# aai-institute/USFlows

Measured on AMD Instinct MI355X. Metric: log_prob samples/sec (whole node), 32-layer 784-dim flow, batch 65536, higher is better.
Workload: dtype f32 (GEMMs as bf16x3 split on the bf16 MFMA: 24 significant bits, fp32 accumulate); 1 GPU; BASELINE cfg2: USFlow in_dims=[784], 32 additive coupling blocks, ConditionalDenseNN[256, 256]+LeakyReLU(0.01), lu_transform=1, householder=0, affine_conjugation=False, Laplace(0,1) base; log_prob of 65536 rows per GPU (65536 over 1 GPU(s)) resident in HBM; conditioned synthetic parameters (seed 100, alpha 0.1); rows_per_gpu=65536, global_rows=65536, parallelism=dp1 (single GPU: no collective), fused_coupling=True, gemm_mode=bf16x3, merge_affine=auto -> False; probe (accepted, element-wise, L1) []

## Files before the change

usflows_amd/csrc/usf_planes.hip:

```cpp
#include <stdlib.h>

#include <type_traits>

#include "usf_common.h"

namespace usf {

typedef __bf16 bf16x8 __attribute__((ext_vector_type(8)));
typedef _Float16 f16x8 __attribute__((ext_vector_type(8)));
typedef unsigned u32x4 __attribute__((ext_vector_type(4)));
#define USF_F16_GUARD 65000.0f
#define USF_PL_LOAD_A(ptr) (*(ptr))
#define USF_PL_STORE_C(v, ptr) (*(ptr) = (v))

template <int NPL> struct Planes;
template <> struct Planes<3> {
  typedef bf16x8 vec;
  static __device__ __forceinline__ f32x4 mfma(vec a, vec b, f32x4 c) { return __builtin_amdgcn_mfma_f32_16x16x32_bf16(a, b, c, 0, 0, 0); }
  static __device__ __forceinline__ void split(const float (&x)[8], vec (&o)[3]) {
#pragma unroll
    for (int j = 0; j < 8; ++j) {
      const __bf16 h = (__bf16)x[j];
      const float r = x[j] - (float)h;
      const __bf16 m = (__bf16)r;
      const float r2 = r - (float)m;
      o[0][j] = h; o[1][j] = m; o[2][j] = (__bf16)r2;
    }
  }
};
template <> struct Planes<2> {
  typedef f16x8 vec;
  static __device__ __forceinline__ f32x4 mfma(vec a, vec b, f32x4 c) { return __builtin_amdgcn_mfma_f32_16x16x32_f16(a, b, c, 0, 0, 0); }
  static __device__ __forceinline__ void split(const float (&x)[8], vec (&o)[2]) {
#pragma unroll
    for (int j = 0; j < 8; ++j) {
      const _Float16 h = (_Float16)x[j];
      const float r = x[j] - (float)h;
      o[0][j] = h; o[1][j] = (_Float16)r;
    }
  }
};

__host__ __device__ __forceinline__ int plane_feature_of_slot(int s) { return 16 * ((s & 7) >> 2) + 4 * (s >> 3) + (s & 3); }

template <int NPL>
__global__ __launch_bounds__(256) void pack_planes_kernel(const float* __restrict__ src, int64_t ld, int M, int npanels,
                                                          int nkb, const int32_t* __restrict__ idx,
                                                          const float* __restrict__ pre_div,
                                                          const float* __restrict__ pre_sub, char* __restrict__ dst,
                                                          int32_t* __restrict__ range_flag) {
  typedef Planes<NPL> PT;
  const int lane = threadIdx.x & 63;
  const int lj = lane & 15, lg = lane >> 4;
  const int64_t chunk = (int64_t)blockIdx.x * 4 + (threadIdx.x >> 6);
  if (chunk >= (int64_t)npanels * nkb) return;
  const int p = (int)(chunk / nkb), kb = (int)(chunk % nkb);
  const int row = 16 * p + lj;
  float x[8];
#pragma unroll
  for (int u = 0; u < 8; ++u) {
    const int l = 32 * kb + 16 * (u >> 2) + 4 * lg + (u & 3);
    const int c = idx[l];
    float v = 0.f;
    if (c >= 0 && row < M) {
      v = src[(int64_t)row * ld + c];
      if (pre_div) v = v / pre_div[l];
      if (pre_sub) v = v - pre_sub[l];
    }
    x[u] = v;
  }
  if (NPL == 2 && range_flag) {
    bool bad = false;
#pragma unroll
    for (int u = 0; u < 8; ++u) bad = bad || !(fabsf(x[u]) < USF_F16_GUARD);
    if (bad) atomicOr(range_flag, 1);
  }
  typename PT::vec o[NPL];
  PT::split(x, o);
  char* out = dst + (chunk * NPL) * 1024 + lane * 16;
#pragma unroll
  for (int q = 0; q < NPL; ++q) *reinterpret_cast<typename PT::vec*>(out + q * 1024) = o[q];
}

template <int NPL, bool GRAD, int NT>
__global__ __launch_bounds__(NT) void pack_planes_rows_kernel(const float* __restrict__ src, int64_t ld, int M, int nkb, int src_cols,
                                                               const int32_t* __restrict__ idx, const float* __restrict__ pre_div,
                                                               const float* __restrict__ pre_sub, char* __restrict__ dst,
                                                               int32_t* __restrict__ range_flag, const float* __restrict__ row_weight,
                                                               const float* __restrict__ loc, const float* __restrict__ scale, int grad_base,
                                                               int vec) {
  typedef Planes<NPL> PT;
  extern __shared__ float tile[];
  const int S = src_cols + 1;
  const int L = 32 * nkb;
  int* const t_idx = reinterpret_cast<int*>(tile + 16 * S);
  float* const t_div = tile + 16 * S + L;
  float* const t_sub = t_div + L;
  const int tid = threadIdx.x, lane = tid & 63, wave = tid >> 6;
  const int p = blockIdx.x;
  for (int e = tid; e < L; e += NT) {
    t_idx[e] = idx[e];
    t_div[e] = pre_div ? pre_div[e] : 1.0f;
    t_sub[e] = pre_sub ? pre_sub[e] : 0.0f;
  }
  auto xform = [&](float v, int c, float w) {
    if (!GRAD) return v;
    const float t = v - loc[c];
    const float sg = (float)((t > 0.f) - (t < 0.f));
    const float g = (grad_base == 1 + USF_BASE_LAPLACE) ? -sg / scale[c] : -t / (scale[c] * scale[c]);
    return g * w;
  };
  if (vec) {
    const int c4n = src_cols >> 2;
    for (int e = tid; e < 16 * c4n; e += NT) {
      const int r = e / c4n, c = 4 * (e - r * c4n);
      const int row = 16 * p + r;
      f32x4 v = {0.f, 0.f, 0.f, 0.f};
      float w = 0.f;
      if (row < M) {
        v = *reinterpret_cast<const f32x4*>(src + (int64_t)row * ld + c);
        if (GRAD) w = row_weight[row];
      }
#pragma unroll
      for (int q = 0; q < 4; ++q) tile[r * S + c + q] = (row < M) ? xform(v[q], c + q, w) : 0.f;
    }
    for (int e = tid; e < 16 * (src_cols & 3); e += NT) {
      const int r = e / (src_cols & 3), c = (src_cols & ~3) + e % (src_cols & 3);
      const int row = 16 * p + r;
      tile[r * S + c] = (row < M) ? xform(src[(int64_t)row * ld + c], c, GRAD ? row_weight[row] : 0.f) : 0.f;
    }
  } else {
    for (int e = tid; e < 16 * src_cols; e += NT) {
      const int r = e / src_cols, c = e - r * src_cols;
      const int row = 16 * p + r;
      tile[r * S + c] = (row < M) ? xform(src[(int64_t)row * ld + c], c, GRAD ? row_weight[row] : 0.f) : 0.f;
    }
  }
  __syncthreads();
  const int lj = lane & 15, lg = lane >> 4;
  const bool row_live = 16 * p + lj < M;
  const bool has_div = pre_div != nullptr, has_sub = pre_sub != nullptr;
  bool bad = false;
  for (int kb = wave; kb < nkb; kb += NT / 64) {
    float x[8];
#pragma unroll
    for (int u = 0; u < 8; ++u) {
      const int l = 32 * kb + 16 * (u >> 2) + 4 * lg + (u & 3);
      const int c = t_idx[l];
      float v = 0.f;
      if (c >= 0 && row_live) {
        v = tile[lj * S + c];
        if (has_div) v = v / t_div[l];
        if (has_sub) v = v - t_sub[l];
      }
      x[u] = v;
    }
    if (NPL == 2) {
#pragma unroll
      for (int u = 0; u < 8; ++u) bad = bad || !(fabsf(x[u]) < USF_F16_GUARD);
    }
    typename PT::vec o[NPL];
    PT::split(x, o);
    char* out = dst + ((int64_t)((int64_t)p * nkb + kb) * NPL) * 1024 + lane * 16;
#pragma unroll
    for (int q = 0; q < NPL; ++q) *reinterpret_cast<typename PT::vec*>(out + q * 1024) = o[q];
  }
  if (NPL == 2 && range_flag && bad) atomicOr(range_flag, 1);
}

int pack_planes(const usf_pack_planes_desc* d, hipStream_t stream) {
  if (!d) { set_error("usf_pack_planes_f32: null descriptor"); return -1; }
  if (d->M < 0 || d->nkb <= 0 || d->M > 0x7fffffff || d->nkb > 0x7fffff || d->ld < 1) { set_error("usf_pack_planes_f32: bad sizes"); return -2; }
  if (d->M == 0) return 0;
  if (!d->src || !d->idx || !d->planes) { set_error("usf_pack_planes_f32: null pointer"); return -1; }
  if (!aligned16(d->planes)) { set_error("usf_pack_planes_f32: planes must be 16-byte aligned"); return -2; }
  if (d->format != USF_PLANES_BF16X3 && d->format != USF_PLANES_F16X2) { set_error("usf_pack_planes_f32: unknown format %d", d->format); return -2; }
  const int64_t npanels = (d->M + 15) / 16;
  const int64_t chunks = npanels * d->nkb;
  const int64_t blocks = (chunks + 3) / 4;
  if (blocks > 0x7fffffffLL) { set_error("usf_pack_planes_f32: grid too large"); return -3; }
  if (d->grad_base != 0) {
    if (d->src_cols <= 0 || !d->row_weight || !d->loc || !d->scale || d->format != USF_PLANES_BF16X3 ||
        (d->grad_base != 1 + USF_BASE_LAPLACE && d->grad_base != 1 + USF_BASE_NORMAL)) {
      set_error("usf_pack_planes_f32: grad_base needs src_cols, row_weight, loc, scale, the bf16x3 format and a Laplace / Normal base");
      return -2;
    }
  }
  const int rows_env = (int)tuning("pack_rows", 1);
  const size_t lds = ((size_t)16 * (size_t)(d->src_cols + 1) + (size_t)3 * 32 * (size_t)d->nkb) * sizeof(float);
  if (d->src_cols > 0 && d->src_cols <= d->ld && lds <= 65536 && (rows_env || d->grad_base != 0)) {
    const int vec = (aligned16(d->src) && (d->ld & 3) == 0) ? 1 : 0;
    char* out = reinterpret_cast<char*>(d->planes);
    const int wide = (int)tuning("pack_wide", 1);
#define USF_PPR(NPL_, GRAD_, NT_) hipLaunchKernelGGL((pack_planes_rows_kernel<NPL_, GRAD_, NT_>), dim3((unsigned)npanels), dim3(NT_), lds, stream, \
                             d->src, d->ld, (int)d->M, (int)d->nkb, (int)d->src_cols, d->idx, d->pre_div, d->pre_sub, out, d->range_flag,  \
                             d->row_weight, d->loc, d->scale, (int)d->grad_base, vec)
#define USF_PPW(NPL_, GRAD_) do { if (wide) USF_PPR(NPL_, GRAD_, 512); else USF_PPR(NPL_, GRAD_, 256); } while (0)
    if (d->grad_base != 0) USF_PPW(3, true);
    else if (d->format == USF_PLANES_F16X2) USF_PPW(2, false);
    else USF_PPW(3, false);
#undef USF_PPW
#undef USF_PPR
    return check_launch("usf_pack_planes_f32");
  }
  if (d->grad_base != 0) { set_error("usf_pack_planes_f32: grad_base needs 16 (src_cols + 1) floats to fit 64 KB of LDS"); return -2; }
  if (d->format == USF_PLANES_F16X2)
    hipLaunchKernelGGL(pack_planes_kernel<2>, dim3((unsigned)blocks), dim3(256), 0, stream, d->src, d->ld, (int)d->M, (int)npanels,
                       (int)d->nkb, d->idx, d->pre_div, d->pre_sub, reinterpret_cast<char*>(d->planes), d->range_flag);
  else
    hipLaunchKernelGGL(pack_planes_kernel<3>, dim3((unsigned)blocks), dim3(256), 0, stream, d->src, d->ld, (int)d->M, (int)npanels,
                       (int)d->nkb, d->idx, d->pre_div, d->pre_sub, reinterpret_cast<char*>(d->planes), d->range_flag);
  return check_launch("usf_pack_planes_f32");
}

struct PlArgs {
  const char* A; const char* Wp; const float* bias; const float* post_mul;
  const char* R; char* Cp; float* Cf;
  int64_t ldc, plane_stride;
  int ldwp, wrows;
  int M, npanels;
  int a_nkb, a_kb0, nk;
  int c_nkb, c_kb0, c_kbn;
  int N, nbm, nbn, nvb;
  float res_sign, slope; int act;
  int32_t* range_flag;
  int skip_dead;
  const float* b_tab; float* b_part; int b_stride; int b_base;
  char* S; int s_kb0, s_kbn, s_both0, s_bothn;
  unsigned long long* clk;
  unsigned long long* dbg;
  unsigned long long* span;
};

template <int NPL, int TN, bool F32OUT, bool SIDE = false>
__global__ __launch_bounds__(512, 2) void gemm_planes_kernel(const PlArgs p) {
  typedef Planes<NPL> PT;
  typedef typename PT::vec vec8;
  constexpr int NT = 512;
  constexpr int BN = TN * 32;
  constexpr int FT = 2 * TN;
  constexpr unsigned CHB = NPL * 1024u;
  constexpr int CS = BN;
  constexpr int NSLOT = NPL * 4 * BN;
  constexpr int NWV = (NSLOT + NT - 1) / NT;
  constexpr int STG = NPL * 4 * CS * 4;
  constexpr int NB = 3;
  static_assert(NWV * NT - NSLOT <= NSLOT, "surplus threads wrap once");
  __shared__ __attribute__((aligned(16))) float wring[NB * STG];

  const int tid0 = threadIdx.x;
#ifdef USF_STAMP
  if (p.span && tid0 == 0) atomicMin(p.span, __builtin_amdgcn_s_memrealtime());
#endif
  unsigned long long clk_c0 = 0, clk_r0 = 0;
#ifndef USF_NO_CLOCK
  if (p.clk) { clk_c0 = __builtin_amdgcn_s_memtime(); clk_r0 = __builtin_amdgcn_s_memrealtime(); }
#endif

  for (int bid = blockIdx.x; bid < p.nvb; bid += gridDim.x) {
  int tid = tid0;
  asm volatile("" : "+v"(tid));
  const int lane = tid & 63;
  const int wave = tid >> 6;
  const int lj = lane & 15, lg = lane >> 4;
  const int xcd = bid & 7;
  const int seq = bid >> 3;
  const int pg = (seq / p.nbn) * 8 + xcd;
  const int bn = seq % p.nbn;
  if (pg >= p.nbm) continue;
  if (bid != (int)blockIdx.x) __syncthreads();
  const int n0 = bn * BN;
  int pw[2];
  pw[0] = pg * 16 + wave * 2;
  pw[1] = pw[0] + 1;

  bool dead = false;
  if (p.skip_dead && bn == p.nbn - 1 && n0 + BN <= p.wrows) {
    const int spr = 4 * p.nk;
    const int nscan = NPL * 16 * spr;
    const char* const wz = p.Wp + 2 * ((int64_t)(n0 + BN - 16) * p.ldwp);
    unsigned nz = 0;
    for (int e0 = tid; e0 < nscan; e0 += 4 * NT) {
      u32x4 v[4];
#pragma unroll
      for (int i = 0; i < 4; ++i) {
        const int e = min(e0 + i * NT, nscan - 1);
        const int pl = e / (16 * spr), rem = e - pl * (16 * spr);
        const int r = rem / spr, c = rem - r * spr;
        v[i] = *reinterpret_cast<const u32x4*>(wz + 2 * (pl * p.plane_stride + (int64_t)r * p.ldwp + 8 * c));
      }
#pragma unroll
      for (int i = 0; i < 4; ++i) nz |= v[i][0] | v[i][1] | v[i][2] | v[i][3];
    }
    dead = __builtin_amdgcn_readfirstlane(__syncthreads_or(nz != 0)) == 0;
  }
  auto tile = [&](auto dead_c) {
  unsigned aoff[2];
#pragma unroll
  for (int b = 0; b < 2; ++b)
    aoff[b] = ((unsigned)min(pw[b], p.npanels - 1) * (unsigned)p.a_nkb + (unsigned)p.a_kb0) * CHB + (unsigned)lane * 16u;
  auto issue_a = [&](int kb, vec8 (&dst)[2][NPL]) {
#pragma unroll
    for (int b = 0; b < 2; ++b)
#pragma unroll
      for (int q = 0; q < NPL; ++q)
        dst[b][q] = USF_PL_LOAD_A(reinterpret_cast<const vec8*>(p.A + (aoff[b] + (unsigned)kb * CHB + (unsigned)q * 1024u)));
  };

  unsigned wsrc[NWV];
  int wdst[NWV];
#pragma unroll
  for (int i = 0; i < NWV; ++i) {
    const int idx = tid + NT * i;
    const int idc = (idx < NSLOT) ? idx : idx - NSLOT;
    const int pl = idc / (4 * BN), rem = idc % (4 * BN);
    const int r = rem >> 2, ch = rem & 3;
    wsrc[i] = (unsigned)(2 * (pl * p.plane_stride + (int64_t)min(n0 + r, p.wrows - 1) * p.ldwp + 8 * ch));
    wdst[i] = 4 * ((pl * 4 + ch) * CS + (r ^ (2 * ch)));
  }
  auto issue_w = [&](int k0, f32x4 (&dst)[NWV]) {
#pragma unroll
    for (int i = 0; i < NWV; ++i) dst[i] = *reinterpret_cast<const f32x4*>(p.Wp + (wsrc[i] + 2u * (unsigned)k0));
  };
  auto store_w = [&](float* wb, const f32x4 (&src)[NWV]) {
#pragma unroll
    for (int i = 0; i < NWV; ++i) *reinterpret_cast<f32x4*>(wb + wdst[i]) = src[i];
  };

  f32x4 acc[FT][2];
  const f32x4 zero4 = {0.f, 0.f, 0.f, 0.f};
#pragma unroll
  for (int ft = 0; ft < FT; ++ft) {
    f32x4 bv = zero4;
    if (p.bias) bv = *reinterpret_cast<const f32x4*>(p.bias + min(n0 + ft * 16 + 4 * lg, p.wrows - 4));
    acc[ft][0] = bv;
    acc[ft][1] = bv;
  }

#ifdef USF_STAMP
#define PSTAMP(v) unsigned long long v = __builtin_amdgcn_s_memtime(); __builtin_amdgcn_sched_barrier(0)
#else
#define PSTAMP(v)
#endif
  PSTAMP(t0);
#ifdef USF_STAMP
  const unsigned long long rt0 = __builtin_amdgcn_s_memrealtime();
#endif
  vec8 pa[2][NPL], pb[2][NPL];
  vec8 fr[2][NPL], f2[2][NPL];
  f32x4 wst[NWV];
  const int nslab = p.nk;
  auto ks = [&](int s_) { return s_; };
  issue_w(ks(0) * 32, wst);
  store_w(wring, wst);
  issue_a(ks(0), pa);
  issue_w(ks(min(1, nslab - 1)) * 32, wst);
  __syncthreads();
  const float* const wl0 = wring + 4 * (lg * CS + (lj ^ (2 * lg)));
  auto read_pair = [&](const float* wl, int pr, vec8 (&f)[2][NPL]) {
#pragma unroll
    for (int q = 0; q < NPL; ++q) {
      f[0][q] = *reinterpret_cast<const vec8*>(wl + 4 * (q * 4 * CS + (2 * pr) * 16));
      f[1][q] = *reinterpret_cast<const vec8*>(wl + 4 * (q * 4 * CS + (2 * pr + 1) * 16));
    }
  };
  auto read_half = [&](const float* wl, int pr, vec8 (&f)[2][NPL]) {
#pragma unroll
    for (int q = 0; q < NPL; ++q) f[0][q] = *reinterpret_cast<const vec8*>(wl + 4 * (q * 4 * CS + (2 * pr) * 16));
  };
  read_pair(wl0, 0, fr);

  constexpr int NPR = (NPL == 3) ? 6 : 3;
  constexpr int NP = TN;
  constexpr int MID = (NP - 1) / 2;
  constexpr int NLD = 2 * NPL;
  constexpr int LPP = (NLD + MID) / (MID + 1);
#define USF_MM(FT_, W, P)                                        \
  acc[FT_][0] = PT::mfma(W, cur[0][P], acc[FT_][0]);             \
  acc[FT_][1] = PT::mfma(W, cur[1][P], acc[FT_][1])
  static_assert(NP - 1 > MID + 1, "the last pair runs behind the barrier and carries no global loads");
  auto mm_pair = [&](auto dead_c, int pr, const vec8 (&f)[2][NPL], const vec8 (&cur)[2][NPL]) {
    const int ft = 2 * pr;
    if (decltype(dead_c)::value && pr == NP - 1) {
      if constexpr (NPL == 3) {
        USF_MM(ft, f[0][2], 0); USF_MM(ft, f[0][1], 1); USF_MM(ft, f[0][0], NPL - 1); USF_MM(ft, f[0][1], 0);
        USF_MM(ft, f[0][0], 1); USF_MM(ft, f[0][0], 0);
      } else {
        USF_MM(ft, f[0][1], 0); USF_MM(ft, f[0][0], 1); USF_MM(ft, f[0][0], 0);
      }
    } else if constexpr (NPL == 3) {
      USF_MM(ft, f[0][2], 0); USF_MM(ft + 1, f[1][2], 0); USF_MM(ft, f[0][1], 1); USF_MM(ft + 1, f[1][1], 1);
      USF_MM(ft, f[0][0], NPL - 1); USF_MM(ft + 1, f[1][0], NPL - 1); USF_MM(ft, f[0][1], 0); USF_MM(ft + 1, f[1][1], 0);
      USF_MM(ft, f[0][0], 1); USF_MM(ft + 1, f[1][0], 1); USF_MM(ft, f[0][0], 0); USF_MM(ft + 1, f[1][0], 0);
    } else {
      USF_MM(ft, f[0][1], 0); USF_MM(ft + 1, f[1][1], 0); USF_MM(ft, f[0][0], 1); USF_MM(ft + 1, f[1][0], 1);
      USF_MM(ft, f[0][0], 0); USF_MM(ft + 1, f[1][0], 0);
    }
  };
#if defined(USF_STAMP) && USF_STAMP >= 2
  unsigned long long ph[4] = {0, 0, 0, 0};
#define LSTAMP(v) PSTAMP(v)
#define LACC(i, a, b) ph[i] += (b) - (a)
#else
#define LSTAMP(v)
#define LACC(i, a, b)
#endif
  auto slab = [&](auto dead_c, int s, int ring_s, const vec8 (&cur)[2][NPL], vec8 (&nxt)[2][NPL], vec8 (&fA)[2][NPL], vec8 (&fB)[2][NPL]) {
    constexpr bool DEAD = decltype(dead_c)::value;
    LSTAMP(l0);
    const int ring_n = (ring_s == 2) ? 0 : ring_s + 1;
    const float* wl = wl0 + ring_s * STG;
    const float* wln = wl0 + ring_n * STG;
    auto read_next = [&](int pr, vec8 (&f)[2][NPL]) {
      if (DEAD && pr + 1 == NP - 1) read_half(wl, pr + 1, f); else read_pair(wl, pr + 1, f);
    };
    float* wb = wring + ring_n * STG;
    issue_a(ks(min(s + 1, nslab - 1)), nxt);
#pragma unroll
    for (int pr = 0; pr <= MID; ++pr) {
      if (pr & 1) { if (pr + 1 < NP) read_next(pr, fA); mm_pair(dead_c, pr, fB, cur); }
      else        { if (pr + 1 < NP) read_next(pr, fB); mm_pair(dead_c, pr, fA, cur); }
      if (pr == MID) store_w(wb, wst);
      __builtin_amdgcn_sched_group_barrier(0x100, 2 * NPL, 0);
      if (pr < MID) {
        __builtin_amdgcn_sched_group_barrier(0x008, 2 * NPR, 0);
        if (pr * LPP < NLD) __builtin_amdgcn_sched_group_barrier(0x020, LPP, 0);
        __builtin_amdgcn_sched_group_barrier(0x008, 2 * NPR, 0);
      } else {
        constexpr int MPS = (4 * NPR) / (NWV + 1);
#pragma unroll
        for (int i = 0; i < NWV; ++i) {
          __builtin_amdgcn_sched_group_barrier(0x008, MPS, 0);
          __builtin_amdgcn_sched_group_barrier(0x200, 1, 0);
        }
        __builtin_amdgcn_sched_group_barrier(0x008, 4 * NPR - NWV * MPS, 0);
      }
    }
    __builtin_amdgcn_sched_barrier(0);
    LSTAMP(l1);
    LSTAMP(l2);
    __syncthreads();
    __builtin_amdgcn_sched_barrier(0);
    LSTAMP(l3);
    issue_w(ks(min(s + 2, nslab - 1)) * 32, wst);
#pragma unroll
    for (int pr = MID + 1; pr < NP; ++pr) {
      if (pr & 1) { if (pr + 1 < NP) read_next(pr, fA); else read_pair(wln, 0, fA); mm_pair(dead_c, pr, fB, cur); }
      else        { if (pr + 1 < NP) read_next(pr, fB); else read_pair(wln, 0, fB); mm_pair(dead_c, pr, fA, cur); }
      if (DEAD && pr + 1 == NP - 1) __builtin_amdgcn_sched_group_barrier(0x100, NPL, 0);
      else __builtin_amdgcn_sched_group_barrier(0x100, 2 * NPL, 0);
      if (pr == MID + 1) {
        __builtin_amdgcn_sched_group_barrier(0x008, 2 * NPR, 0);
        __builtin_amdgcn_sched_group_barrier(0x020, NWV, 0);
        __builtin_amdgcn_sched_group_barrier(0x008, 2 * NPR, 0);
      } else if (DEAD && pr == NP - 1) {
        __builtin_amdgcn_sched_group_barrier(0x008, 2 * NPR, 0);
      } else {
        __builtin_amdgcn_sched_group_barrier(0x008, 4 * NPR, 0);
      }
    }
    __builtin_amdgcn_sched_barrier(0);
    LSTAMP(l4);
    LACC(0, l0, l1); LACC(1, l1, l2); LACC(2, l2, l3); LACC(3, l3, l4);
  };
  PSTAMP(t1);
    int s = 0, ring = 0;
    for (; s + 2 <= nslab; s += 2) {
      slab(dead_c, s, ring, pa, pb, fr, f2);
      ring = (ring == 2) ? 0 : ring + 1;
      if (NP & 1) slab(dead_c, s + 1, ring, pb, pa, f2, fr); else slab(dead_c, s + 1, ring, pb, pa, fr, f2);
      ring = (ring == 2) ? 0 : ring + 1;
    }
    if (s < nslab) slab(dead_c, s, ring, pa, pb, fr, f2);
  PSTAMP(t2);

  bool bad = false;
  if (p.act == USF_ACT_LEAKY_RELU) {
#pragma unroll
    for (int ft = 0; ft < FT; ++ft)
#pragma unroll
      for (int b = 0; b < 2; ++b)
#pragma unroll
        for (int j = 0; j < 4; ++j) acc[ft][b][j] = act_apply(acc[ft][b][j], USF_ACT_LEAKY_RELU, p.slope);
  }
  if (F32OUT) {
    const bool vec_ok = ((p.ldc & 3) == 0) && ((reinterpret_cast<uintptr_t>(p.Cf) & 15u) == 0);
#pragma unroll
    for (int b = 0; b < 2; ++b) {
      const int row = 16 * pw[b] + lj;
      float bsum = 0.f;
#pragma unroll
      for (int ft = 0; ft < FT; ++ft) {
        const int col = n0 + 16 * ft + 4 * lg;
        f32x4 v = acc[ft][b];
        if (p.post_mul) v = v * *reinterpret_cast<const f32x4*>(p.post_mul + min(col, p.wrows - 4));
        if (p.b_part) {
          const float* t = p.b_tab + min(col, p.b_stride - 4);
          const f32x4 bl = *reinterpret_cast<const f32x4*>(t);
          const f32x4 bi = *reinterpret_cast<const f32x4*>(t + p.b_stride);
          const f32x4 bc = *reinterpret_cast<const f32x4*>(t + 2 * p.b_stride);
#pragma unroll
          for (int j = 0; j < 4; ++j) {
            const float d = (v[j] - bl[j]) * bi[j];
            const float term = (p.b_base == USF_BASE_LAPLACE) ? bc[j] - fabsf(d) : bc[j] - 0.5f * d * d;
            bsum += (col + j < p.N) ? term : 0.f;
          }
        }
        if (NPL == 2 && row < p.M && col < p.N) {
#pragma unroll
          for (int j = 0; j < 4; ++j) bad = bad || (col + j < p.N && !(fabsf(v[j]) < 3.0e38f));
        }
        if (p.Cf != nullptr && row < p.M && col < p.N) {
          float* dst = p.Cf + (int64_t)row * p.ldc + col;
          if (vec_ok && col + 3 < p.N) {
            *reinterpret_cast<f32x4*>(dst) = v;
          } else {
#pragma unroll
            for (int j = 0; j < 4; ++j)
              if (col + j < p.N) dst[j] = v[j];
          }
        }
      }
      if (p.b_part) {
        bsum += __shfl_xor(bsum, 16);
        bsum += __shfl_xor(bsum, 32);
        if (lg == 0 && row < p.M) p.b_part[(int64_t)row * 8 + bn] = bsum;
      }
    }
  } else {
#pragma unroll
    for (int t = 0; t < TN; ++t) {
      const int kbo = bn * TN + t;
      const bool to_side = SIDE && (unsigned)(kbo - p.s_kb0) < (unsigned)p.s_kbn;
      const bool to_planes = !to_side || (unsigned)(kbo - p.s_both0) < (unsigned)p.s_bothn;
#pragma unroll
      for (int b = 0; b < 2; ++b) {
        if (kbo < p.c_kbn && pw[b] < p.npanels) {
          const size_t off = (((size_t)pw[b] * p.c_nkb + (p.c_kb0 + kbo)) * NPL) * 1024 + (size_t)lane * 16;
          float x[8];
#pragma unroll
          for (int u = 0; u < 8; ++u) x[u] = acc[2 * t + (u >> 2)][b][u & 3];
          if constexpr (SIDE) {
            if (to_side) {
              const unsigned soff = ((unsigned)pw[b] * (unsigned)p.s_kbn + (unsigned)(kbo - p.s_kb0)) * 2048u + (unsigned)lane * 32u;
              f32x4 s0 = {x[0], x[1], x[2], x[3]}, s1 = {x[4], x[5], x[6], x[7]};
              if constexpr (NPL == 2) {
                bool sb = false;
#pragma unroll
                for (int u = 0; u < 8; ++u) sb = sb || (16 * pw[b] + lj < p.M && !(fabsf(x[u]) < USF_F16_GUARD));
                bad = bad || sb;
                vec8 so[NPL];
                PT::split(x, so);
#pragma unroll
                for (int u = 0; u < 4; ++u) {
                  s0[u] = (float)so[0][u] + (float)so[1][u];
                  s1[u] = (float)so[0][4 + u] + (float)so[1][4 + u];
                }
              }
              *reinterpret_cast<f32x4*>(p.S + soff) = s0;
              *reinterpret_cast<f32x4*>(p.S + (soff + 16u)) = s1;
            }
            if (!to_planes) continue;
          }
          if (p.R) {
            vec8 r[NPL];
#pragma unroll
            for (int q = 0; q < NPL; ++q) r[q] = *reinterpret_cast<const vec8*>(p.R + off + q * 1024);
#pragma unroll
            for (int u = 0; u < 8; ++u) {
              float rv = (float)r[0][u] + (float)r[1][u];
              if (NPL == 3) rv = rv + (float)r[NPL - 1][u];
              x[u] = rv + p.res_sign * x[u];
            }
          }
          if (NPL == 2) {
#pragma unroll
            for (int u = 0; u < 8; ++u) bad = bad || (16 * pw[b] + lj < p.M && !(fabsf(x[u]) < USF_F16_GUARD));
          }
          vec8 o[NPL];
          PT::split(x, o);
#ifdef USF_NOSTORE
          if (o[0][0] == (decltype(o[0][0] + o[0][0]))1234.5f && o[1][1] == (decltype(o[0][0] + o[0][0]))77.f)
#endif
          {
#pragma unroll
            for (int q = 0; q < NPL; ++q) USF_PL_STORE_C(o[q], reinterpret_cast<vec8*>(p.Cp + off + q * 1024));
          }
        }
      }
    }
  }
  if (NPL == 2 && p.range_flag && bad) atomicOr(p.range_flag, 1);
#ifdef USF_STAMP
  PSTAMP(t3);
  if (p.dbg && lane == 0) {
    unsigned long long* o = p.dbg + (size_t)((bid % 2048) * 8 + wave) * 8;
    o[0] = t1 - t0; o[1] = t2 - t1; o[2] = t3 - t2; o[3] = t3 - t0; o[4] = 1; o[5] = __builtin_amdgcn_s_memrealtime() - rt0;
    o[6] = rt0; o[7] = __builtin_amdgcn_s_memrealtime();
#if USF_STAMP >= 2
    unsigned long long* o2 = p.dbg + 16384 * 8 + (size_t)((bid % 2048) * 8 + wave) * 8;
    for (int i = 0; i < 4; ++i) o2[i] = ph[i];
#endif
  }
#endif
  };
  if (dead) tile(std::true_type()); else tile(std::false_type());
#undef USF_MM
  }
#ifdef USF_STAMP
  if (p.span && tid0 == 0) atomicMax(p.span + 1, __builtin_amdgcn_s_memrealtime());
#endif
#ifndef USF_NO_CLOCK
  if (p.clk && tid0 == 0) {
    atomicAdd(p.clk, __builtin_amdgcn_s_memtime() - clk_c0);
    atomicAdd(p.clk + 1, __builtin_amdgcn_s_memrealtime() - clk_r0);
  }
#endif
}

#ifdef USF_STAMP
unsigned long long* g_pdbg = nullptr;
unsigned long long* g_pspan = nullptr;
#endif

template <int NPL, int TN>
static int launch_planes(PlArgs a, bool f32out, hipStream_t stream) {
  const bool side = a.S != nullptr;
  constexpr int BN = TN * 32;
  a.nbm = (a.npanels + 15) / 16;
  a.nbn = f32out ? (a.N + BN - 1) / BN : (a.c_kbn + TN - 1) / TN;
  int64_t grid = (((int64_t)a.nbm + 7) / 8) * 8 * a.nbn;
  if (grid > 0x7fffffffLL) { set_error("usf_gemm_planes: grid too large"); return -3; }
  a.nvb = (int)grid;
  const int persist = (int)tuning("planes_persist", 1);
  int cus = device_cu_count();
  cus = (cus / 8) * 8 > 0 ? (cus / 8) * 8 : 8;
  if (persist && grid > cus) grid = cus;
  if (f32out) hipLaunchKernelGGL((gemm_planes_kernel<NPL, TN, true>), dim3((unsigned)grid), dim3(512), 0, stream, a);
  else if (side) hipLaunchKernelGGL((gemm_planes_kernel<NPL, TN, false, true>), dim3((unsigned)grid), dim3(512), 0, stream, a);
  else hipLaunchKernelGGL((gemm_planes_kernel<NPL, TN, false>), dim3((unsigned)grid), dim3(512), 0, stream, a);
  return check_launch("usf_gemm_planes");
}

int gemm_planes_tn(int64_t nblk) {
  const int64_t pad5 = (nblk + 4) / 5 * 5 - nblk, pad4 = (nblk + 3) / 4 * 4 - nblk;
  return pad4 < pad5 ? 4 : 5;
}

int gemm_planes_variant(const usf_gemm_planes_desc* d) {
  if (!d || d->M <= 0) return 0;
  const bool f32out = d->C_f32 != nullptr || d->base_part != nullptr;
  const int64_t nblk = f32out ? (d->N + 31) / 32 : d->c_kbn;
  if (nblk <= 0) return 0;
  return 5000 + 10 * gemm_planes_tn(nblk) + (f32out ? 1 : 0);
}

int gemm_planes_side(const usf_gemm_planes_desc* d, void* side, int64_t side_kb0, int64_t side_kbn, int64_t both_kb0,
                     int64_t both_kbn, hipStream_t stream) {
  if (!d) { set_error("usf_gemm_planes_bf16x3: null descriptor"); return -1; }
  if (d->M < 0 || d->M > 0x7fffffff || d->nk <= 0 || d->a_nkb <= 0 || d->a_kb0 < 0 || d->a_kb0 + d->nk > d->a_nkb ||
      d->w_rows < 4 || d->w_rows > 0x7fffffff) {
    set_error("usf_gemm_planes_bf16x3: bad sizes (M=%lld nk=%lld a_nkb=%lld a_kb0=%lld w_rows=%lld)", (long long)d->M,
              (long long)d->nk, (long long)d->a_nkb, (long long)d->a_kb0, (long long)d->w_rows);
    return -2;
  }
  if (d->M == 0) return 0;
  const bool f32out = d->C_f32 != nullptr || d->base_part != nullptr;
  if (!d->A || !d->W_planes || (!f32out && !d->C_planes)) { set_error("usf_gemm_planes_bf16x3: null A / W / C"); return -1; }
  if (f32out && d->C_planes) { set_error("usf_gemm_planes_bf16x3: give C_planes or C_f32, not both"); return -2; }
  if (!aligned16(d->A) || !aligned16(d->W_planes) || (d->C_planes && !aligned16(d->C_planes)) ||
      (d->residual && !aligned16(d->residual)) || (d->bias && !aligned16(d->bias)) || (d->post_mul && !aligned16(d->post_mul))) {
    set_error("usf_gemm_planes_bf16x3: pointers must be 16-byte aligned");
    return -2;
  }
  if ((d->ldw & 7) || d->ldw < 32 * d->nk || (d->w_rows & 3)) { set_error("usf_gemm_planes_bf16x3: ldw must be a multiple of 8 and >= 32 nk; w_rows a multiple of 4"); return -2; }
  if (d->act != USF_ACT_NONE && d->act != USF_ACT_LEAKY_RELU) { set_error("usf_gemm_planes_bf16x3: bad act"); return -2; }
  const int64_t npanels = (d->M + 15) / 16;
  if (d->format != USF_PLANES_BF16X3 && d->format != USF_PLANES_F16X2) { set_error("usf_gemm_planes_bf16x3: unknown format %d", d->format); return -2; }
  const int64_t npl = d->format == USF_PLANES_F16X2 ? 2 : 3;
  if (npanels * d->a_nkb * npl * 1024 >= (1LL << 32) || 2 * npl * d->w_plane_stride >= (1LL << 32)) {
    set_error("usf_gemm_planes_bf16x3: operand larger than the kernel's 32-bit offsets");
    return -3;
  }
  PlArgs a;
  a.A = reinterpret_cast<const char*>(d->A); a.Wp = reinterpret_cast<const char*>(d->W_planes);
  a.bias = d->bias; a.post_mul = d->post_mul; a.R = reinterpret_cast<const char*>(d->residual);
  a.Cp = reinterpret_cast<char*>(d->C_planes); a.Cf = d->C_f32; a.ldc = d->ldc; a.plane_stride = d->w_plane_stride;
  a.ldwp = (int)d->ldw; a.wrows = (int)d->w_rows; a.M = (int)d->M; a.npanels = (int)npanels;
  a.a_nkb = (int)d->a_nkb; a.a_kb0 = (int)d->a_kb0; a.nk = (int)d->nk;
  a.c_nkb = (int)d->c_nkb; a.c_kb0 = (int)d->c_kb0; a.c_kbn = (int)d->c_kbn; a.N = (int)d->N;
  a.res_sign = d->res_sign; a.slope = d->slope; a.act = d->act; a.nbm = a.nbn = a.nvb = 0;
  a.range_flag = d->range_flag;
  a.skip_dead = (int)tuning("planes_skip_dead", 1);
  a.b_tab = d->base_tab; a.b_part = d->base_part; a.b_stride = (int)d->base_tab_stride; a.b_base = d->base;
  a.dbg = nullptr; a.span = nullptr;
  a.S = nullptr; a.s_kb0 = a.s_kbn = a.s_both0 = a.s_bothn = 0;
  if (side) {
    if (f32out || d->residual) { set_error("usf_gemm_planes_side: the side output needs planes output and no residual"); return -2; }
    if (!aligned16(side)) { set_error("usf_gemm_planes_side: side must be 16-byte aligned"); return -2; }
    if (side_kbn <= 0 || side_kb0 < 0 || side_kb0 + side_kbn > d->c_kbn || both_kbn < 0 ||
        (both_kbn > 0 && (both_kb0 < side_kb0 || both_kb0 + both_kbn > side_kb0 + side_kbn))) {
      set_error("usf_gemm_planes_side: bad block ranges (side %lld + %lld of c_kbn=%lld, both %lld + %lld)", (long long)side_kb0,
                (long long)side_kbn, (long long)d->c_kbn, (long long)both_kb0, (long long)both_kbn);
      return -2;
    }
    if (npanels * side_kbn * 2048 >= (1LL << 32)) { set_error("usf_gemm_planes_side: side buffer larger than the kernel's 32-bit offsets"); return -3; }
    a.S = reinterpret_cast<char*>(side); a.s_kb0 = (int)side_kb0; a.s_kbn = (int)side_kbn;
    a.s_both0 = (int)both_kb0; a.s_bothn = (int)both_kbn;
  }
  a.clk = clock_buffer();
#ifdef USF_STAMP
  a.dbg = g_pdbg; a.span = g_pspan;
  if (g_pspan) g_pspan += 2;
#endif
  int64_t nblk;
  if (f32out) {
    if (d->N <= 0 || d->N > d->w_rows || d->ldc < d->N) { set_error("usf_gemm_planes_bf16x3: bad N / ldc for fp32 output"); return -2; }
    if (d->residual) { set_error("usf_gemm_planes_bf16x3: residual needs planes output"); return -2; }
    nblk = (d->N + 31) / 32;
    if (d->base_part) {
      if (!d->base_tab || !aligned16(d->base_tab) || (d->base_tab_stride & 3) || d->base_tab_stride < ((d->N + 3) & ~(int64_t)3) ||
          d->base_tab_stride > 0x7fffffff || (d->base != USF_BASE_LAPLACE && d->base != USF_BASE_NORMAL)) {
        set_error("usf_gemm_planes_bf16x3: base density in the epilogue needs the tables of usf_base_tables_f32 (16-byte aligned, "
                  "stride a multiple of 4 and >= N) and base = USF_BASE_LAPLACE / USF_BASE_NORMAL");
        return -2;
      }
    }
  } else {
    if (d->base_part) { set_error("usf_gemm_planes_bf16x3: base_part needs the fp32-output form"); return -2; }
    if (d->c_kbn <= 0 || d->c_kb0 < 0 || d->c_kb0 + d->c_kbn > d->c_nkb || d->c_kbn * 32 > d->w_rows) {
      set_error("usf_gemm_planes_bf16x3: bad output block range (c_kb0=%lld c_kbn=%lld c_nkb=%lld w_rows=%lld)",
                (long long)d->c_kb0, (long long)d->c_kbn, (long long)d->c_nkb, (long long)d->w_rows);
      return -2;
    }
    if (npanels * d->c_nkb * npl * 1024 >= (1LL << 40)) { set_error("usf_gemm_planes_bf16x3: output too large"); return -3; }
    nblk = d->c_kbn;
  }
  const int force = (int)tuning("planes_tn", 0);
  const int tn = (force == 4 || force == 5) ? force : gemm_planes_tn(nblk);
  if (d->base_part && (d->N + 32 * tn - 1) / (32 * tn) > 8) {
    set_error("usf_gemm_planes_bf16x3: base_part holds 8 column blocks per row (N <= 1024)");
    return -2;
  }
  if (npl == 2) return tn == 4 ? launch_planes<2, 4>(a, f32out, stream) : launch_planes<2, 5>(a, f32out, stream);
  return tn == 4 ? launch_planes<3, 4>(a, f32out, stream) : launch_planes<3, 5>(a, f32out, stream);
}

int gemm_planes(const usf_gemm_planes_desc* d, hipStream_t stream) { return gemm_planes_side(d, nullptr, 0, 0, 0, 0, stream); }

}
```

Before: 3.605 million samples/s.

## Stream persistent GEMM tiles with cross-tile prefetch and rolled epilogue

Adds a streaming mode to the persistent planes GEMM kernel that is on by default for non-f32 outputs. The A and W prefetch queues run continuously across successive tiles instead of restarting at each tile, and the epilogue (activation, residual, split, store) is interleaved into the last slab's MFMA pairs. Bias is staged once in LDS and the dead-column scan runs once per block. This removes the per-tile pipeline drain, prologue and barrier, at the cost of more register pressure, extra LDS, and more complex scheduling that could hurt occupancy or correctness.

```diff
diff --git a/usflows_amd/csrc/usf_planes.hip b/usflows_amd/csrc/usf_planes.hip
--- a/usflows_amd/csrc/usf_planes.hip
+++ b/usflows_amd/csrc/usf_planes.hip
@@ -232,11 +232,14 @@
   unsigned long long* span;
 };
 
-template <int NPL, int TN, bool F32OUT, bool SIDE = false>
+constexpr int PL_BIAS_LDS = 4096;
+
+template <int NPL, int TN, bool F32OUT, bool SIDE = false, int STREAM = 0>
 __global__ __launch_bounds__(512, 2) void gemm_planes_kernel(const PlArgs p) {
   typedef Planes<NPL> PT;
   typedef typename PT::vec vec8;
   constexpr int NT = 512;
+  constexpr bool ROLL = STREAM == 2;
   constexpr int BN = TN * 32;
   constexpr int FT = 2 * TN;
   constexpr unsigned CHB = NPL * 1024u;
@@ -247,6 +250,7 @@
   constexpr int NB = 3;
   static_assert(NWV * NT - NSLOT <= NSLOT, "surplus threads wrap once");
   __shared__ __attribute__((aligned(16))) float wring[NB * STG];
+  __shared__ f32x4 bias_s[STREAM ? PL_BIAS_LDS / 4 : 1];
 
   const int tid0 = threadIdx.x;
 #ifdef USF_STAMP
@@ -257,6 +261,54 @@
   if (p.clk) { clk_c0 = __builtin_amdgcn_s_memtime(); clk_r0 = __builtin_amdgcn_s_memrealtime(); }
 #endif
 
+  auto vb_pg = [&](int b) { return ((b >> 3) / p.nbn) * 8 + (b & 7); };
+  auto vb_bn = [&](int b) { return (b >> 3) % p.nbn; };
+  auto vb_next = [&](int b) { return b < p.nvb - (int)gridDim.x && vb_pg(b + (int)gridDim.x) < p.nbm; };
+  auto scan_dead = [&](int tid, int n0) {
+    const int spr = 4 * p.nk;
+    const int nscan = NPL * 16 * spr;
+    const char* const wz = p.Wp + 2 * ((int64_t)(n0 + BN - 16) * p.ldwp);
+    unsigned nz = 0;
+    for (int e0 = tid; e0 < nscan; e0 += 4 * NT) {
+      u32x4 v[4];
+#pragma unroll
+      for (int i = 0; i < 4; ++i) {
+        const int e = min(e0 + i * NT, nscan - 1);
+        const int pl = e / (16 * spr), rem = e - pl * (16 * spr);
+        const int r = rem / spr, c = rem - r * spr;
+        v[i] = *reinterpret_cast<const u32x4*>(wz + 2 * (pl * p.plane_stride + (int64_t)r * p.ldwp + 8 * c));
+      }
+#pragma unroll
+      for (int i = 0; i < 4; ++i) nz |= v[i][0] | v[i][1] | v[i][2] | v[i][3];
+    }
+    return __builtin_amdgcn_readfirstlane(__syncthreads_or(nz != 0)) == 0;
+  };
+  typename PT::vec pa[2][NPL], pb[2][NPL];
+  typename PT::vec fr[2][NPL], f2[2][NPL];
+  f32x4 wst[NWV];
+  f32x4 acc[FT][2];
+  unsigned aoff[2];
+  unsigned wsrc[NWV];
+  int wdst[NWV];
+  int ring = 0;
+  int wq_bid = 0, wq_s = 0, aq_bid = 0, aq_s = 0;
+  bool sdead = false;
+  if constexpr (STREAM) {
+    if ((int)blockIdx.x < p.nvb && vb_pg(blockIdx.x) < p.nbm) {
+      const f32x4 z4 = {0.f, 0.f, 0.f, 0.f};
+      for (int i = tid0; i < p.nbn * (BN / 4); i += NT)
+        bias_s[i] = p.bias ? *reinterpret_cast<const f32x4*>(p.bias + min(4 * i, p.wrows - 4)) : z4;
+      __syncthreads();
+      bool has_last = false;
+      if (p.skip_dead && p.nbn * BN <= p.wrows) {
+        for (int b = blockIdx.x; !has_last; b += gridDim.x) {
+          has_last = vb_bn(b) == p.nbn - 1;
+          if (!vb_next(b)) break;
+        }
+      }
+      if (has_last) sdead = scan_dead(tid0, (p.nbn - 1) * BN);
+    }
+  }
   for (int bid = blockIdx.x; bid < p.nvb; bid += gridDim.x) {
   int tid = tid0;
   asm volatile("" : "+v"(tid));
@@ -267,38 +319,23 @@
   const int seq = bid >> 3;
   const int pg = (seq / p.nbn) * 8 + xcd;
   const int bn = seq % p.nbn;
-  if (pg >= p.nbm) continue;
-  if (bid != (int)blockIdx.x) __syncthreads();
+  if (pg >= p.nbm) { if constexpr (STREAM) break; else continue; }
+  const bool first = bid == (int)blockIdx.x;
+  if (!STREAM && !first) __syncthreads();
   const int n0 = bn * BN;
   int pw[2];
   pw[0] = pg * 16 + wave * 2;
   pw[1] = pw[0] + 1;
 
   bool dead = false;
-  if (p.skip_dead && bn == p.nbn - 1 && n0 + BN <= p.wrows) {
-    const int spr = 4 * p.nk;
-    const int nscan = NPL * 16 * spr;
-    const char* const wz = p.Wp + 2 * ((int64_t)(n0 + BN - 16) * p.ldwp);
-    unsigned nz = 0;
-    for (int e0 = tid; e0 < nscan; e0 += 4 * NT) {
-      u32x4 v[4];
-#pragma unroll
-      for (int i = 0; i < 4; ++i) {
-        const int e = min(e0 + i * NT, nscan - 1);
-        const int pl = e / (16 * spr), rem = e - pl * (16 * spr);
-        const int r = rem / spr, c = rem - r * spr;
-        v[i] = *reinterpret_cast<const u32x4*>(wz + 2 * (pl * p.plane_stride + (int64_t)r * p.ldwp + 8 * c));
-      }
-#pragma unroll
-      for (int i = 0; i < 4; ++i) nz |= v[i][0] | v[i][1] | v[i][2] | v[i][3];
-    }
-    dead = __builtin_amdgcn_readfirstlane(__syncthreads_or(nz != 0)) == 0;
-  }
+  if constexpr (STREAM) dead = sdead && bn == p.nbn - 1;
+  else if (p.skip_dead && bn == p.nbn - 1 && n0 + BN <= p.wrows) dead = scan_dead(tid, n0);
   auto tile = [&](auto dead_c) {
-  unsigned aoff[2];
-#pragma unroll
-  for (int b = 0; b < 2; ++b)
-    aoff[b] = ((unsigned)min(pw[b], p.npanels - 1) * (unsigned)p.a_nkb + (unsigned)p.a_kb0) * CHB + (unsigned)lane * 16u;
+  auto set_aoff = [&](int t, int pgx) {
+#pragma unroll
+    for (int b = 0; b < 2; ++b)
+      aoff[b] = ((unsigned)min(pgx * 16 + (t >> 6) * 2 + b, p.npanels - 1) * (unsigned)p.a_nkb + (unsigned)p.a_kb0) * CHB + (unsigned)(t & 63) * 16u;
+  };
   auto issue_a = [&](int kb, vec8 (&dst)[2][NPL]) {
 #pragma unroll
     for (int b = 0; b < 2; ++b)
@@ -307,17 +344,17 @@
         dst[b][q] = USF_PL_LOAD_A(reinterpret_cast<const vec8*>(p.A + (aoff[b] + (unsigned)kb * CHB + (unsigned)q * 1024u)));
   };
 
-  unsigned wsrc[NWV];
-  int wdst[NWV];
-#pragma unroll
-  for (int i = 0; i < NWV; ++i) {
-    const int idx = tid + NT * i;
-    const int idc = (idx < NSLOT) ? idx : idx - NSLOT;
-    const int pl = idc / (4 * BN), rem = idc % (4 * BN);
-    const int r = rem >> 2, ch = rem & 3;
-    wsrc[i] = (unsigned)(2 * (pl * p.plane_stride + (int64_t)min(n0 + r, p.wrows - 1) * p.ldwp + 8 * ch));
-    wdst[i] = 4 * ((pl * 4 + ch) * CS + (r ^ (2 * ch)));
-  }
+  auto set_wsrc = [&](int t, int n0x) {
+#pragma unroll
+    for (int i = 0; i < NWV; ++i) {
+      const int idx = t + NT * i;
+      const int idc = (idx < NSLOT) ? idx : idx - NSLOT;
+      const int pl = idc / (4 * BN), rem = idc % (4 * BN);
+      const int r = rem >> 2, ch = rem & 3;
+      wsrc[i] = (unsigned)(2 * (pl * p.plane_stride + (int64_t)min(n0x + r, p.wrows - 1) * p.ldwp + 8 * ch));
+      wdst[i] = 4 * ((pl * 4 + ch) * CS + (r ^ (2 * ch)));
+    }
+  };
   auto issue_w = [&](int k0, f32x4 (&dst)[NWV]) {
 #pragma unroll
     for (int i = 0; i < NWV; ++i) dst[i] = *reinterpret_cast<const f32x4*>(p.Wp + (wsrc[i] + 2u * (unsigned)k0));
@@ -327,12 +364,13 @@
     for (int i = 0; i < NWV; ++i) *reinterpret_cast<f32x4*>(wb + wdst[i]) = src[i];
   };
 
-  f32x4 acc[FT][2];
   const f32x4 zero4 = {0.f, 0.f, 0.f, 0.f};
 #pragma unroll
   for (int ft = 0; ft < FT; ++ft) {
+    if (ROLL && !first) break;
     f32x4 bv = zero4;
-    if (p.bias) bv = *reinterpret_cast<const f32x4*>(p.bias + min(n0 + ft * 16 + 4 * lg, p.wrows - 4));
+    if constexpr (STREAM) bv = bias_s[bn * (BN / 4) + ft * 4 + lg];
+    else if (p.bias) bv = *reinterpret_cast<const f32x4*>(p.bias + min(n0 + ft * 16 + 4 * lg, p.wrows - 4));
     acc[ft][0] = bv;
     acc[ft][1] = bv;
   }
@@ -346,16 +384,16 @@
 #ifdef USF_STAMP
   const unsigned long long rt0 = __builtin_amdgcn_s_memrealtime();
 #endif
-  vec8 pa[2][NPL], pb[2][NPL];
-  vec8 fr[2][NPL], f2[2][NPL];
-  f32x4 wst[NWV];
   const int nslab = p.nk;
-  auto ks = [&](int s_) { return s_; };
-  issue_w(ks(0) * 32, wst);
-  store_w(wring, wst);
-  issue_a(ks(0), pa);
-  issue_w(ks(min(1, nslab - 1)) * 32, wst);
-  __syncthreads();
+  auto own_tid = [&]() { int t = tid0; asm volatile("" : "+v"(t)); return t; };
+  auto w_adv = [&]() {
+    if (wq_s + 1 < nslab) ++wq_s;
+    else if (vb_next(wq_bid)) { wq_bid += (int)gridDim.x; wq_s = 0; set_wsrc(own_tid(), vb_bn(wq_bid) * BN); }
+  };
+  auto a_adv = [&]() {
+    if (aq_s + 1 < nslab) ++aq_s;
+    else if (vb_next(aq_bid)) { aq_bid += (int)gridDim.x; aq_s = 0; set_aoff(own_tid(), vb_pg(aq_bid)); }
+  };
   const float* const wl0 = wring + 4 * (lg * CS + (lj ^ (2 * lg)));
   auto read_pair = [&](const float* wl, int pr, vec8 (&f)[2][NPL]) {
 #pragma unroll
@@ -368,7 +406,18 @@
 #pragma unroll
     for (int q = 0; q < NPL; ++q) f[0][q] = *reinterpret_cast<const vec8*>(wl + 4 * (q * 4 * CS + (2 * pr) * 16));
   };
-  read_pair(wl0, 0, fr);
+  if (!STREAM || first) {
+    if constexpr (STREAM) { wq_bid = aq_bid = bid; wq_s = aq_s = 0; }
+    set_aoff(tid, pg);
+    set_wsrc(tid, n0);
+    issue_w(0, wst);
+    store_w(wring, wst);
+    issue_a(0, pa);
+    if constexpr (STREAM) { w_adv(); issue_w(wq_s * 32, wst); }
+    else issue_w(min(1, nslab - 1) * 32, wst);
+    __syncthreads();
+    read_pair(wl0, 0, fr);
+  }
 
   constexpr int NPR = (NPL == 3) ? 6 : 3;
   constexpr int NP = TN;
@@ -405,8 +454,92 @@
 #define LSTAMP(v)
 #define LACC(i, a, b)
 #endif
-  auto slab = [&](auto dead_c, int s, int ring_s, const vec8 (&cur)[2][NPL], vec8 (&nxt)[2][NPL], vec8 (&fA)[2][NPL], vec8 (&fB)[2][NPL]) {
+  bool bad = false;
+  const int bn_nx = (ROLL && vb_next(bid)) ? vb_bn(bid + (int)gridDim.x) : bn;
+  auto epi_line = [&](int t) {
+    if constexpr (ROLL) {
+      if (p.act == USF_ACT_LEAKY_RELU) {
+#pragma unroll
+        for (int h = 0; h < 2; ++h)
+#pragma unroll
+          for (int b = 0; b < 2; ++b)
+#pragma unroll
+            for (int j = 0; j < 4; ++j) acc[2 * t + h][b][j] = act_apply(acc[2 * t + h][b][j], USF_ACT_LEAKY_RELU, p.slope);
+      }
+    }
+    {
+      const int kbo = bn * TN + t;
+      const bool to_side = SIDE && (unsigned)(kbo - p.s_kb0) < (unsigned)p.s_kbn;
+      const bool to_planes = !to_side || (unsigned)(kbo - p.s_both0) < (unsigned)p.s_bothn;
+#pragma unroll
+      for (int b = 0; b < 2; ++b) {
+        if constexpr (ROLL) __builtin_amdgcn_sched_barrier(0);
+        if (kbo < p.c_kbn && pw[b] < p.npanels) {
+          const size_t off = (((size_t)pw[b] * p.c_nkb + (p.c_kb0 + kbo)) * NPL) * 1024 + (size_t)lane * 16;
+          float x[8];
+#pragma unroll
+          for (int u = 0; u < 8; ++u) x[u] = acc[2 * t + (u >> 2)][b][u & 3];
+          if constexpr (SIDE) {
+            if (to_side) {
+              const unsigned soff = ((unsigned)pw[b] * (unsigned)p.s_kbn + (unsigned)(kbo - p.s_kb0)) * 2048u + (unsigned)lane * 32u;
+              f32x4 s0 = {x[0], x[1], x[2], x[3]}, s1 = {x[4], x[5], x[6], x[7]};
+              if constexpr (NPL == 2) {
+                bool sb = false;
+#pragma unroll
+                for (int u = 0; u < 8; ++u) sb = sb || (16 * pw[b] + lj < p.M && !(fabsf(x[u]) < USF_F16_GUARD));
+                bad = bad || sb;
+                vec8 so[NPL];
+                PT::split(x, so);
+#pragma unroll
+                for (int u = 0; u < 4; ++u) {
+                  s0[u] = (float)so[0][u] + (float)so[1][u];
+                  s1[u] = (float)so[0][4 + u] + (float)so[1][4 + u];
+                }
+              }
+              *reinterpret_cast<f32x4*>(p.S + soff) = s0;
+              *reinterpret_cast<f32x4*>(p.S + (soff + 16u)) = s1;
+            }
+            if (!to_planes) continue;
+          }
+          if (p.R) {
+            vec8 r[NPL];
+#pragma unroll
+            for (int q = 0; q < NPL; ++q) r[q] = *reinterpret_cast<const vec8*>(p.R + off + q * 1024);
+#pragma unroll
+            for (int u = 0; u < 8; ++u) {
+              float rv = (float)r[0][u] + (float)r[1][u];
+              if (NPL == 3) rv = rv + (float)r[NPL - 1][u];
+              x[u] = rv + p.res_sign * x[u];
+            }
+          }
+          if (NPL == 2) {
+#pragma unroll
+            for (int u = 0; u < 8; ++u) bad = bad || (16 * pw[b] + lj < p.M && !(fabsf(x[u]) < USF_F16_GUARD));
+          }
+          vec8 o[NPL];
+          PT::split(x, o);
+#ifdef USF_NOSTORE
+          if (o[0][0] == (decltype(o[0][0] + o[0][0]))1234.5f && o[1][1] == (decltype(o[0][0] + o[0][0]))77.f)
+#endif
+          {
+#pragma unroll
+            for (int q = 0; q < NPL; ++q) USF_PL_STORE_C(o[q], reinterpret_cast<vec8*>(p.Cp + off + q * 1024));
+          }
+        }
+      }
+    }
+    if constexpr (ROLL) {
+#pragma unroll
+      for (int h = 0; h < 2; ++h) {
+        const f32x4 bv = bias_s[bn_nx * (BN / 4) + (2 * t + h) * 4 + lg];
+        acc[2 * t + h][0] = bv;
+        acc[2 * t + h][1] = bv;
+      }
+    }
+  };
+  auto slab = [&](auto dead_c, auto last_c, int kb_a, int k0_w, int ring_s, const vec8 (&cur)[2][NPL], vec8 (&nxt)[2][NPL], vec8 (&fA)[2][NPL], vec8 (&fB)[2][NPL]) {
     constexpr bool DEAD = decltype(dead_c)::value;
+    constexpr bool LAST = decltype(last_c)::value;
     LSTAMP(l0);
     const int ring_n = (ring_s == 2) ? 0 : ring_s + 1;
     const float* wl = wl0 + ring_s * STG;
@@ -415,7 +548,7 @@
       if (DEAD && pr + 1 == NP - 1) read_half(wl, pr + 1, f); else read_pair(wl, pr + 1, f);
     };
     float* wb = wring + ring_n * STG;
-    issue_a(ks(min(s + 1, nslab - 1)), nxt);
+    issue_a(kb_a, nxt);
 #pragma unroll
     for (int pr = 0; pr <= MID; ++pr) {
       if (pr & 1) { if (pr + 1 < NP) read_next(pr, fA); mm_pair(dead_c, pr, fB, cur); }
@@ -435,6 +568,7 @@
         }
         __builtin_amdgcn_sched_group_barrier(0x008, 4 * NPR - NWV * MPS, 0);
       }
+      if (LAST && pr >= 1) { __builtin_amdgcn_sched_barrier(0); epi_line(pr - 1); __builtin_amdgcn_sched_barrier(0); }
     }
     __builtin_amdgcn_sched_barrier(0);
     LSTAMP(l1);
@@ -442,9 +576,20 @@
     __syncthreads();
     __builtin_amdgcn_sched_barrier(0);
     LSTAMP(l3);
-    issue_w(ks(min(s + 2, nslab - 1)) * 32, wst);
+    issue_w(k0_w, wst);
 #pragma unroll
     for (int pr = MID + 1; pr < NP; ++pr) {
+      if (STREAM && pr == NP - 1) {
+        auto last = [&](auto dc) {
+          if (pr & 1) { read_pair(wln, 0, fA); mm_pair(dc, pr, fB, cur); }
+          else        { read_pair(wln, 0, fB); mm_pair(dc, pr, fA, cur); }
+          __builtin_amdgcn_sched_group_barrier(0x100, 2 * NPL, 0);
+          __builtin_amdgcn_sched_group_barrier(0x008, decltype(dc)::value ? 2 * NPR : 4 * NPR, 0);
+        };
+        if (dead) last(std::true_type()); else last(std::false_type());
+        if (LAST) { __builtin_amdgcn_sched_barrier(0); epi_line(pr - 1); }
+        break;
+      }
       if (pr & 1) { if (pr + 1 < NP) read_next(pr, fA); else read_pair(wln, 0, fA); mm_pair(dead_c, pr, fB, cur); }
       else        { if (pr + 1 < NP) read_next(pr, fB); else read_pair(wln, 0, fB); mm_pair(dead_c, pr, fA, cur); }
       if (DEAD && pr + 1 == NP - 1) __builtin_amdgcn_sched_group_barrier(0x100, NPL, 0);
@@ -458,24 +603,52 @@
       } else {
         __builtin_amdgcn_sched_group_barrier(0x008, 4 * NPR, 0);
       }
+      if (LAST) { __builtin_amdgcn_sched_barrier(0); epi_line(pr - 1); __builtin_amdgcn_sched_barrier(0); }
     }
     __builtin_amdgcn_sched_barrier(0);
     LSTAMP(l4);
     LACC(0, l0, l1); LACC(1, l1, l2); LACC(2, l2, l3); LACC(3, l3, l4);
   };
   PSTAMP(t1);
-    int s = 0, ring = 0;
-    for (; s + 2 <= nslab; s += 2) {
-      slab(dead_c, s, ring, pa, pb, fr, f2);
+    int s = 0;
+    if constexpr (!STREAM) ring = 0;
+    auto step = [&](auto last_c, int s_, const vec8 (&cur)[2][NPL], vec8 (&nxt)[2][NPL], vec8 (&fA)[2][NPL], vec8 (&fB)[2][NPL]) {
+      if constexpr (STREAM) {
+        w_adv();
+        a_adv();
+        slab(dead_c, last_c, aq_s, wq_s * 32, ring, cur, nxt, fA, fB);
+      } else {
+        slab(dead_c, last_c, min(s_ + 1, nslab - 1), min(s_ + 2, nslab - 1) * 32, ring, cur, nxt, fA, fB);
+      }
       ring = (ring == 2) ? 0 : ring + 1;
-      if (NP & 1) slab(dead_c, s + 1, ring, pb, pa, f2, fr); else slab(dead_c, s + 1, ring, pb, pa, fr, f2);
-      ring = (ring == 2) ? 0 : ring + 1;
-    }
-    if (s < nslab) slab(dead_c, s, ring, pa, pb, fr, f2);
+    };
+    const std::false_type inner;
+    const std::integral_constant<bool, ROLL> last;
+    for (; s + 2 <= nslab - (ROLL ? 1 : 0); s += 2) {
+      step(inner, s, pa, pb, fr, f2);
+      if (NP & 1) step(inner, s + 1, pb, pa, f2, fr); else step(inner, s + 1, pb, pa, fr, f2);
+    }
+    auto to_front = [&]() {
+#pragma unroll
+      for (int b = 0; b < 2; ++b)
+#pragma unroll
+        for (int q = 0; q < NPL; ++q) {
+          pa[b][q] = pb[b][q];
+          if (NP & 1) fr[b][q] = f2[b][q];
+        }
+    };
+    if (ROLL && s + 2 == nslab) {
+      step(inner, s, pa, pb, fr, f2);
+      to_front();
+      ++s;
+    }
+    if (s < nslab) {
+      step(last, s, pa, pb, fr, f2);
+      if constexpr (STREAM) to_front();
+    }
   PSTAMP(t2);
 
-  bool bad = false;
-  if (p.act == USF_ACT_LEAKY_RELU) {
+  if (!ROLL && p.act == USF_ACT_LEAKY_RELU) {
 #pragma unroll
     for (int ft = 0; ft < FT; ++ft)
 #pragma unroll
@@ -528,66 +701,11 @@
       }
     }
   } else {
-#pragma unroll
-    for (int t = 0; t < TN; ++t) {
-      const int kbo = bn * TN + t;
-      const bool to_side = SIDE && (unsigned)(kbo - p.s_kb0) < (unsigned)p.s_kbn;
-      const bool to_planes = !to_side || (unsigned)(kbo - p.s_both0) < (unsigned)p.s_bothn;
-#pragma unroll
-      for (int b = 0; b < 2; ++b) {
-        if (kbo < p.c_kbn && pw[b] < p.npanels) {
-          const size_t off = (((size_t)pw[b] * p.c_nkb + (p.c_kb0 + kbo)) * NPL) * 1024 + (size_t)lane * 16;
-          float x[8];
-#pragma unroll
-          for (int u = 0; u < 8; ++u) x[u] = acc[2 * t + (u >> 2)][b][u & 3];
-          if constexpr (SIDE) {
-            if (to_side) {
-              const unsigned soff = ((unsigned)pw[b] * (unsigned)p.s_kbn + (unsigned)(kbo - p.s_kb0)) * 2048u + (unsigned)lane * 32u;
-              f32x4 s0 = {x[0], x[1], x[2], x[3]}, s1 = {x[4], x[5], x[6], x[7]};
-              if constexpr (NPL == 2) {
-                bool sb = false;
-#pragma unroll
-                for (int u = 0; u < 8; ++u) sb = sb || (16 * pw[b] + lj < p.M && !(fabsf(x[u]) < USF_F16_GUARD));
-                bad = bad || sb;
-                vec8 so[NPL];
-                PT::split(x, so);
-#pragma unroll
-                for (int u = 0; u < 4; ++u) {
-                  s0[u] = (float)so[0][u] + (float)so[1][u];
-                  s1[u] = (float)so[0][4 + u] + (float)so[1][4 + u];
-                }
-              }
-              *reinterpret_cast<f32x4*>(p.S + soff) = s0;
-              *reinterpret_cast<f32x4*>(p.S + (soff + 16u)) = s1;
-            }
-            if (!to_planes) continue;
-          }
-          if (p.R) {
-            vec8 r[NPL];
-#pragma unroll
-            for (int q = 0; q < NPL; ++q) r[q] = *reinterpret_cast<const vec8*>(p.R + off + q * 1024);
-#pragma unroll
-            for (int u = 0; u < 8; ++u) {
-              float rv = (float)r[0][u] + (float)r[1][u];
-              if (NPL == 3) rv = rv + (float)r[NPL - 1][u];
-              x[u] = rv + p.res_sign * x[u];
-            }
-          }
-          if (NPL == 2) {
-#pragma unroll
-            for (int u = 0; u < 8; ++u) bad = bad || (16 * pw[b] + lj < p.M && !(fabsf(x[u]) < USF_F16_GUARD));
-          }
-          vec8 o[NPL];
-          PT::split(x, o);
-#ifdef USF_NOSTORE
-          if (o[0][0] == (decltype(o[0][0] + o[0][0]))1234.5f && o[1][1] == (decltype(o[0][0] + o[0][0]))77.f)
-#endif
-          {
-#pragma unroll
-            for (int q = 0; q < NPL; ++q) USF_PL_STORE_C(o[q], reinterpret_cast<vec8*>(p.Cp + off + q * 1024));
-          }
-        }
-      }
+    if constexpr (ROLL) {
+      epi_line(TN - 1);
+    } else {
+#pragma unroll
+      for (int t = 0; t < TN; ++t) epi_line(t);
     }
   }
   if (NPL == 2 && p.range_flag && bad) atomicOr(p.range_flag, 1);
@@ -604,7 +722,7 @@
   }
 #endif
   };
-  if (dead) tile(std::true_type()); else tile(std::false_type());
+  if (!STREAM && dead) tile(std::true_type()); else tile(std::false_type());
 #undef USF_MM
   }
 #ifdef USF_STAMP
@@ -635,8 +753,16 @@
   const int persist = (int)tuning("planes_persist", 1);
   int cus = device_cu_count();
   cus = (cus / 8) * 8 > 0 ? (cus / 8) * 8 : 8;
+  const int cap = (int)tuning("planes_grid", 0);
+  if (cap >= 8) cus = cap / 8 * 8 < cus ? cap / 8 * 8 : cus;
   if (persist && grid > cus) grid = cus;
-  if (f32out) hipLaunchKernelGGL((gemm_planes_kernel<NPL, TN, true>), dim3((unsigned)grid), dim3(512), 0, stream, a);
+  const int knob = (int)tuning("planes_stream", 2);
+  const int strm = (f32out || (int64_t)a.nbn * BN > PL_BIAS_LDS || knob < 0 || knob > 2) ? 0 : knob;
+#define USF_PLS(SIDE_, STRM_) hipLaunchKernelGGL((gemm_planes_kernel<NPL, TN, false, SIDE_, STRM_>), dim3((unsigned)grid), dim3(512), 0, stream, a)
+  if (strm == 2) { if (side) USF_PLS(true, 2); else USF_PLS(false, 2); }
+  else if (strm == 1) { if (side) USF_PLS(true, 1); else USF_PLS(false, 1); }
+#undef USF_PLS
+  else if (f32out) hipLaunchKernelGGL((gemm_planes_kernel<NPL, TN, true>), dim3((unsigned)grid), dim3(512), 0, stream, a);
   else if (side) hipLaunchKernelGGL((gemm_planes_kernel<NPL, TN, false, true>), dim3((unsigned)grid), dim3(512), 0, stream, a);
   else hipLaunchKernelGGL((gemm_planes_kernel<NPL, TN, false>), dim3((unsigned)grid), dim3(512), 0, stream, a);
   return check_launch("usf_gemm_planes");
```

Result: no change. 3.636 million samples/s (median of 6 runs) (+0.9%).
